# Roy-Kid/ADMP

Hardware: AMD Instinct MI355X
Metric: ns/day (electrostatics get_forces per 1 fs step, polarizable PME incl. SCF, moving atoms) (higher is better)
Workload: dtype f64; 1 GPU; water_pol_1024 (BASELINE configs[1]): 1024 polarizable MPID waters = 3072 atoms, seeded liquid box L=31.289 A, rc 4 A, f64; n_atoms=3072, n_pairs=42510, pair_list=fixed during the timed steps, parallelism=single GPU

## Files before the change

admp_amd/_lib.py:

```python
import ctypes

import numpy as np
import os

_HERE = os.path.dirname(os.path.abspath(__file__))
LIB_PATH = os.environ.get('ADMP_HIP_LIB') or os.path.join(_HERE, 'lib', 'libadmp_hip.so')

_c = ctypes
_vp, _i32, _i64, _dbl = _c.c_void_p, _c.c_int, _c.c_int64, _c.c_double
_dp = _c.POINTER(_c.c_double)
_ip = _c.POINTER(_c.c_int)

PROTOTYPES = {
    'admp_version': (_c.c_char_p, []),
    'admp_create': (_i32, [_c.POINTER(_vp), _i32, _i32]),
    'admp_destroy': (_i32, [_vp]),
    'admp_last_error': (_c.c_char_p, [_vp]),
    'admp_set_stream': (_i32, [_vp, _vp]),
    'admp_use_default_stream': (_i32, [_vp]),
    'admp_synchronize': (_i32, [_vp]),
    'admp_set_topology': (_i32, [_vp, _i32, _vp, _vp, _vp, _vp, _vp]),
    'admp_set_ewald': (_i32, [_vp, _dbl, _i32, _i32, _i32, _i32, _i32]),
    'admp_set_pairs': (_i32, [_vp, _i64, _vp, _i32]),
    'admp_share_neighbors': (_i32, [_vp, _vp]),
# ... 15 lines not shown
    'admp_pair_program_build': (_i32, [_vp, _c.c_char_p, _i32, _ip]),
    'admp_pair_program_energy_grad': (_i32, [_vp, _i32, _vp, _dp, _vp, _i32, _dp, _dp, _vp, _i32]),
    'admp_disp_param_grad': (_i32, [_vp, _vp, _dp, _vp, _i32, _i32, _dp, _vp]),
    'admp_tt_param_grad': (_i32, [_vp, _vp, _dp, _vp, _i32, _dp, _vp]),
    'admp_thole_sums': (_i32, [_vp, _vp, _dp, _vp, _vp, _vp, _i32, _dp, _dp, _vp, _vp, _vp]),
    'admp_pscale_grad': (_i32, [_vp, _vp, _dp, _vp, _vp, _vp, _i32, _dp, _dp, _vp, _dp]),
    'admp_mscale_grad': (_i32, [_vp, _i32, _vp, _dp, _vp, _i32, _i32, _dp, _i32]),
    'admp_md_bonded': (_i32, [_vp, _vp, _dp, _i32, _vp, _vp, _i32, _vp, _vp, _vp, _vp]),
    'admp_md_kick_drift': (_i32, [_vp, _i32, _vp, _vp, _vp, _vp, _dbl, _dbl, _vp]),
    'admp_neighbor_count': (_i32, [_vp, _i32, _vp, _dp, _dbl, _c.POINTER(_i64)]),
    'admp_neighbor_fill': (_i32, [_vp, _vp]),
    'admp_set_pairs_from_positions': (_i32, [_vp, _vp, _dp, _dbl]),
    'admp_slab_configure': (_i32, [_vp, _i32, _i32]),
    'admp_slab_info': (_i32, [_vp, _c.POINTER(_i64)]),
    'admp_scf_stats': (_i32, [_vp, _c.POINTER(_i64), _i32]),
    'admp_set_comm': (_i32, [_vp, _vp]),
    'admp_slab_home': (_i32, [_vp, _vp, _ip, _ip]),
    'admp_rccl_unique_id': (_i32, [_vp]),
    'admp_rccl_create': (_i32, [_c.POINTER(_vp), _i32, _vp, _i32, _i32]),
    'admp_rccl_destroy': (_i32, [_vp]),
    'admp_rccl_abort': (_i32, [_vp]),
    'admp_rccl_stats': (_i32, [_vp, _c.POINTER(_i64), _c.POINTER(_i64), _i32]),
    'admp_rccl_all_reduce': (_i32, [_vp, _vp, _i64, _i32, _i32, _vp]),
    'admp_rccl_all_to_all_v': (_i32, [_vp, _vp, _c.POINTER(_i64), _vp, _c.POINTER(_i64), _i32, _vp]),
    'admp_rccl_shift': (_i32, [_vp, _vp, _vp, _i64, _i32, _i32, _vp]),
    'admp_rccl_version': (_i32, [_ip]),
    'admp_rccl_last_error': (_c.c_char_p, []),
    'admp_set_comm_rccl': (_i32, [_vp, _vp]),
    'admp_profile_enable': (_i32, [_vp, _i32]),
    'admp_profile_filter': (_i32, [_vp, _c.c_char_p]),
# ... 58 lines not shown
```

admp_amd/csrc/dft_kernels.hip:

```cpp
#include "dft_lines.h"
#include "env.h"

namespace admp {

int dft_tile_cols(int N) { return dft_cols(N, dft_kq(), 0, 0); }
template <class T, int KQ, int JS>
__global__ __launch_bounds__(kDftBlock) void k_dft_z_r2c(int N, int nlines, int NL, int TK, const T* __restrict__ mesh,
                                                        Cx<T>* __restrict__ spec, const Cx<T>* __restrict__ twg,
                                                        long mesh_stride, long spec_stride) {
  mesh += blockIdx.y * mesh_stride;
  spec += blockIdx.y * spec_stride;
  const int H = (N - 1) / 2, Kh = N / 2 + 1;
  Cx<T>* tw = reinterpret_cast<Cx<T>*>(dft_smem);
  Cx<T>* p = tw + N;
  T* x0 = reinterpret_cast<T*>(p + H * NL);
  T* xn = x0 + NL;
  const int line0 = blockIdx.x * NL;
  const int nl = min(NL, nlines - line0);
  for (int t = threadIdx.x; t < N; t += kDftBlock) tw[t] = twg[t];
  for (int t = threadIdx.x; t < H * nl; t += kDftBlock) {
    const int l = t / H, jj = t - l * H;
    const T* x = mesh + (long)(line0 + l) * N;
    const T a = x[1 + jj], b = x[N - 1 - jj];
    p[jj * NL + l] = Cx<T>{a + b, a - b};
// ... 108 lines not shown
    dft_pair_outputs_js<T, SIGN, KQ, JS>(N, k, NC, ab + c, x0[c], xn[c], tw, half, Xk, Xnk);
#pragma unroll
    for (int q = 0; q < KQ; ++q) {
      const int kq = g + q * TK;
      if (kq < Kh) {
        if (JS == 1 || half == 0) spec[base + (long)kq * jstride + c] = Xk[q];
        if ((JS == 1 || half == 1) && kq != 0 && 2 * kq != N) spec[base + (long)(N - kq) * jstride + c] = Xnk[q];
      }
    }
  }
}

template <class T, int KQ, int JS>
__global__ __launch_bounds__(kDftBlock) void k_dft_x_conv(XConvArgs<T> xa) {
  dft_x_conv_body<T, KQ, JS>(xa, blockIdx.x, blockIdx.y, blockIdx.z);
}

template <class T, int KQ, int JS, int NTP>
__global__ __launch_bounds__(kDftBlock) void k_dft_x_mix(int N, int ncols, int NC, int TK, long jstride, long fixstride,
                                                        int K3, Cx<T>* __restrict__ spec, DftTabs<T> tabs, MixTab mix,
                                                        const Cx<T>* __restrict__ twg, double* energies, int slot,
                                                        long spec_tstride) {
  const int H = (N - 1) / 2, Kh = N / 2 + 1, NCt = NC / NTP;
  PairCx<T>* ab = reinterpret_cast<PairCx<T>*>(dft_smem);
  Cx<T>* tw = reinterpret_cast<Cx<T>*>(ab + H * NC);
  Cx<T>* x0 = tw + N;
  Cx<T>* xn = x0 + NC;
  Cx<T>* S = xn + NC;
  const int col0 = blockIdx.x * NCt;
  const int ncp = min(NCt, ncols - col0);
// ... 463 lines not shown
    KQ_SWITCH((k_dft_strided<T, -1, KQ, JS><<<grid, kDftBlock, sh, st>>>(N, Kh, NC, TK, (long)Kh, (long)K[1] * Kh, sp, t1, ss)))
  }
}
template <class T>
void launch_dft_x_conv(hipStream_t st, const int K[3], const T* tw, T* spec, const DftTabs<T>& tabs, double* energies,
                       int slot, int nb, long spec_stride) {
  const int N = K[0], Kh = K[2] / 2 + 1, H = (N - 1) / 2, TK = dft_tasks(N, dft_kq());
  const int NC = dft_cols(N, dft_kq(), sizeof(PairCx<T>) * (size_t)H + sizeof(Cx<T>) * (size_t)(2 + N), sizeof(Cx<T>) * (size_t)N);
  const size_t sh = sizeof(PairCx<T>) * (size_t)(H * NC) + sizeof(Cx<T>) * (size_t)(N + 2 * NC + N * NC);
  const dim3 grid((Kh + NC - 1) / NC, K[1], nb);
  const XConvArgs<T> xa{N, Kh, NC, TK, (long)K[1] * Kh, (long)Kh, K[2], reinterpret_cast<Cx<T>*>(spec), tabs,
                        reinterpret_cast<const Cx<T>*>(tw), energies, slot, spec_stride / 2};
  KQ_SWITCH((k_dft_x_conv<T, KQ, JS><<<grid, kDftBlock, sh, st>>>(xa)))
}
template <class T>
void launch_dft_x_mix(hipStream_t st, const int K[3], const T* tw, T* spec, const DftTabs<T>& tabs, const MixTab& mix,
                      long spec_stride, double* energies, int slot) {
  const int N = K[0], Kh = K[2] / 2 + 1, H = (N - 1) / 2, TK = dft_tasks(N, dft_kq());
  const int ntp = mix.nt <= 1 ? 1 : (mix.nt == 2 ? 2 : 4);
  int NC = dft_cols(N, dft_kq(), sizeof(PairCx<T>) * (size_t)H + sizeof(Cx<T>) * (size_t)(2 + N), sizeof(Cx<T>) * (size_t)N);
  NC -= NC % ntp;
  if (NC < ntp) NC = ntp;
  const int NCt = NC / ntp;
  const size_t sh = sizeof(PairCx<T>) * (size_t)(H * NC) + sizeof(Cx<T>) * (size_t)(N + 2 * NC + N * NC);
  const dim3 grid((Kh + NCt - 1) / NCt, K[1], 1);
#define XMIX(NTP)                                                                                                          \
  k_dft_x_mix<T, 2, 1, NTP><<<grid, kDftBlock, sh, st>>>(N, Kh, NC, TK, (long)K[1] * Kh, (long)Kh, K[2],                    \
                                                         reinterpret_cast<Cx<T>*>(spec), tabs, mix,                        \
                                                         reinterpret_cast<const Cx<T>*>(tw), energies, slot, spec_stride / 2)
  if (ntp == 1) XMIX(1); else if (ntp == 2) XMIX(2); else XMIX(4);
// ... 33 lines not shown
  }
  auto kern = k_dft_zy_fwd<T, 2, false>;
  if (attr_set[0] < sh) { (void)hipFuncSetAttribute((const void*)kern, hipFuncAttributeMaxDynamicSharedMemorySize, (int)sh); attr_set[0] = sh; }
  kern<<<grid, kZyBlock, sh, st>>>(K[1], K[2], mesh, reinterpret_cast<Cx<T>*>(spec), t1, t2, mesh_stride, spec_stride / 2,
                                   PlaneSpread<T>());
  return false;
}
#undef KQ_SWITCH
#define INST(T)                                                                                   \
  template bool dft_zy_fits<T>(const int*);                                                       \
  template bool dft_zy_spread_fits<T>(const int*, int);                                           \
  template bool launch_dft_zy<T>(hipStream_t, const int*, const T*, T*, T*, int, int, long, long, T*, const PlaneSpread<T>*); \
  template bool launch_dft_z<T>(hipStream_t, const int*, const T*, T*, T*, int, int, long, long, T*); \
  template void launch_dft_y<T>(hipStream_t, const int*, const T*, T*, int, int, long);           \
  template void launch_dft_x_conv<T>(hipStream_t, const int*, const T*, T*, const DftTabs<T>&, double*, int, int, long); \
  template void launch_dft_x_mix<T>(hipStream_t, const int*, const T*, T*, const DftTabs<T>&, const MixTab&, long, double*, int);
INST(float)
INST(double)
#undef INST

}
```

admp_amd/csrc/dft_lines.h:

```cpp
#pragma once
#include "dft_math.h"
#include "launch.h"
#include "reduce.h"

namespace admp {

#ifndef ADMP_DFT_BLOCK
#define ADMP_DFT_BLOCK 256
#endif
constexpr int kDftBlock = ADMP_DFT_BLOCK;
constexpr size_t kDftLdsBudget = 60 * 1024;

static inline int dft_kq() { return 2; }
static inline int dft_js() { return 1; }
static inline int dft_tasks(int N, int KQ) { return (N / 2 + 1 + KQ - 1) / KQ; }
static inline int dft_cols(int N, int KQ, size_t bytes_per_col, size_t fixed_bytes) {
  int nc = (kDftBlock / dft_js()) / dft_tasks(N, KQ);
  if (nc < 1) nc = 1;
  while (nc > 1 && fixed_bytes + bytes_per_col * nc > kDftLdsBudget) --nc;
  return nc;
}

extern __shared__ __align__(32) unsigned char dft_smem[];

// ... 59 lines not shown
    xn[c] = b;
  }
}

template <class T>
struct XConvArgs {
  int N, ncols, NC, TK;
  long jstride, fixstride;
  int K3;
  Cx<T>* spec;
  DftTabs<T> tabs;
  const Cx<T>* twg;
  double* energies;
  int slot;
  long spec_stride;
};
template <class T, int KQ, int JS>
__device__ __forceinline__ void dft_x_conv_body(const XConvArgs<T>& xa, int bx, int by, int bz) {
  const int N = xa.N, ncols = xa.ncols, NC = xa.NC, TK = xa.TK, K3 = xa.K3, slot = xa.slot;
  const long jstride = xa.jstride, fixstride = xa.fixstride;
  const Cx<T>* __restrict__ twg = xa.twg;
  double* energies = xa.energies;
  Cx<T>* __restrict__ spec = xa.spec + bz * xa.spec_stride;
  const T* __restrict__ gtab = xa.tabs.p[bz];
  const int H = (N - 1) / 2, Kh = N / 2 + 1;
  PairCx<T>* ab = reinterpret_cast<PairCx<T>*>(dft_smem);
  Cx<T>* tw = reinterpret_cast<Cx<T>*>(ab + H * NC);
  Cx<T>* x0 = tw + N;
  Cx<T>* xn = x0 + NC;
  Cx<T>* S = xn + NC;
// ... 82 lines not shown
    Cx<T> Xk[KQ], Xnk[KQ];
    dft_pair_outputs_js<T, +1, KQ, JS>(N, k, NC, ab + c, x0[c], xn[c], tw, half, Xk, Xnk);
#pragma unroll
    for (int q = 0; q < KQ; ++q) {
      const int kq = g + q * TK;
      if (kq < Kh) {
        if (JS == 1 || half == 0) spec[base + (long)kq * jstride + c] = Xk[q];
        if ((JS == 1 || half == 1) && kq != 0 && 2 * kq != N) spec[base + (long)(N - kq) * jstride + c] = Xnk[q];
      }
    }
  }
  e = block_reduce_sum<kDftBlock>(e);
  if (threadIdx.x == 0) atomicAdd(&energies[slot], e);
}

}
```

admp_amd/csrc/dft_math.h:

```cpp
#pragma once
#include "pme_math.h"

namespace admp {

template <class T>
struct alignas(2 * sizeof(T)) Cx {
  T re, im;
};
template <class T>
struct alignas(4 * sizeof(T)) PairCx {
  T are, aim, bre, bim;
};

constexpr int kDftReseed = 8;

template <class T>
ADMP_HD Cx<T> cx_mul(Cx<T> a, Cx<T> b) {
  return Cx<T>{a.re * b.re - a.im * b.im, a.re * b.im + a.im * b.re};
}

template <class T>
struct TwStep {
  Cx<T> w, aux;
  T t;
// ... 175 lines not shown

template <class T, int KQ>
ADMP_HD void irdft_pair_outputs(int N, const int* j, int stride, const Cx<T>* p, T X0re, T Xnre, const Cx<T>* tw, T* xj,
                                T* xnj) {
  T P[KQ], R[KQ];
  real_pair_sums<T, KQ>(N, j, stride, p, tw, P, R);
#pragma unroll
  for (int q = 0; q < KQ; ++q) {
    T base = X0re + T(2) * P[q];
    if ((N & 1) == 0) base += (j[q] & 1) ? -Xnre : Xnre;
    xj[q] = base - T(2) * R[q];
    xnj[q] = base + T(2) * R[q];
  }
}

inline int largest_prime_factor(int n) {
  int best = 1;
  for (int p = 2; (long)p * p <= n; ++p)
    while (n % p == 0) {
      best = p;
      n /= p;
    }
  return n > 1 ? (n > best ? n : best) : best;
}

}
```

admp_amd/csrc/engine.hip:

```cpp
#include <hip/hip_runtime.h>
#include <hip/hiprtc.h>
#include <rocfft/rocfft.h>

#include <algorithm>
#include <cmath>
#include <cstdio>
#include <cstring>
#include <map>
#include <memory>
#include <mutex>
#include <set>
#include <string>
#include <functional>
#include <vector>

#include "../../include/admp_hip.h"
#include "dft_math.h"
#include "launch.h"
#include "rccl_comm.h"
#include "scf_policy.h"

using namespace admp;

namespace {
// ... 132 lines not shown
  void c_all_reduce(void* buf, int64_t n, int dtype, int op, int tag) {
    const int rc = rccl ? rccl_all_reduce(rccl, stream, buf, n, dtype, op, tag) : comm.all_reduce(comm.ctx, buf, n, dtype, op, tag);
    if (rc != 0) comm_fail("all_reduce", rc);
  }
  void c_all_to_all_v(const void* send, const int64_t* sc, void* recv, const int64_t* rc_, int dtype, int tag) {
    const int rc = rccl ? rccl_all_to_all_v(rccl, stream, send, sc, recv, rc_, dtype, tag)
                        : comm.all_to_all_v(comm.ctx, send, sc, recv, rc_, dtype, tag);
    if (rc != 0) comm_fail("all_to_all_v", rc);
  }
  void c_shift(const void* send, void* recv, int64_t n, int dtype, int to_next, int tag) {
    const int rc = rccl ? rccl_shift(rccl, stream, send, recv, n, dtype, to_next, tag)
                        : comm.shift(comm.ctx, send, recv, n, dtype, to_next, tag);
    if (rc != 0) comm_fail("shift", rc);
  }
  int64_t scf_stats[8] = {0, 0, 0, 0, 0, 0, 0, 0};
  const void* U_src = nullptr;
  const void* U_src_now = nullptr;
  double cutoff = 0.0;
  int ref_korder = 0;
  int keep_pol_sites = 0;
  int side_stream_on = 1;
  virtual void after_error() {}
  long nbr_gen = 0;
  NbrTable nbr_full;
  bool pruned = false;
  void unprune() {
    if (!pruned) return;
    nbr = nbr_full;
    nbr_full = NbrTable();
    pruned = false;
// ... 347 lines not shown
  const IndTable& wind() const { return cut_on ? cut_ind : ind; }
  long act_gen = 0, act_top_na = -1;
  int act_n = -1;
  bool act_fresh = false;
  long ind_nbr_gen = -1, ind_act_gen = -1;
  long eval_seq = 0, ind_bins_eval = -1, ind_bins_gen = -1;
  int ind_bins_n = -1;
  const int* ind_bins_at = nullptr;
  DevBuf dft_tw;
  DevBuf bases_d;
  bool use_dft = false;
  bool use_pfa = false;
  PfaPlan pfa;
  DevBuf pfa_tw, pfa_fmap, pfa_ptab, gtab_nat;
  struct TabKey { double box[9] = {0}, kappa = -1; int K[3] = {0, 0, 0}, Y0 = 0, ref = 0; bool pfa = false; } tabkey[4];
  static int tab_slot(int which) { return which == 1 ? 0 : (which == 6 ? 1 : (which == 8 ? 2 : 3)); }
  static_assert(kScfChainSteps == E_CHAIN, "one residual word per chained Jacobi step");
  ScfHistory scf;
  bool mono_ok = false;

  ~Engine() override {
    destroy_plans();
    for (DevBuf* b : {&sites, &grad, &pot, &fld_pair, &fld_recip, &field, &energies_d, &s_pos, &s_Q, &s_pol,
                      &s_thole, &s_U, &s_out, &s_dQ, &s_par, &mesh, &spec, &gtabs[0], &gtabs[1], &gtabs[2], &gtabs[3], &fft_work, &binv_d, &scan_scratch, &bin_cells,
                      &bin_sorted, &bin_scan, &home_list, &dft_tw, &bases_d, &vir_d, &act_d, &isites, &mesh2, &act_tmp,
                      &rq_d, &pfa_tw, &pfa_fmap, &pfa_ptab, &gtab_nat, &fx_tw, &bin_cells_ind, &bin_sorted_ind, &srow_d, &onehot_d, &tcount_d, &prune_rowptr, &prune_cnt, &prune_col,
                      &cut_end, &cut_col, &cut_iend, &cut_icol})
      b->release();
    free_topology();
    if (ind.end) (void)hipFree(ind.end);
    if (ind.col) (void)hipFree(ind.col);
    cells.release();
    sl.release();
    free_programs();
    if (Eh) (void)hipHostFree(Eh);
    prof.destroy();
    if (side) { (void)hipStreamSynchronize(side); (void)hipStreamDestroy(side); }
    if (ev_fork) (void)hipEventDestroy(ev_fork);
    if (ev_join) (void)hipEventDestroy(ev_join);
    if (own_stream && stream) (void)hipStreamDestroy(stream);
  }

// ... 404 lines not shown
      { TIMED("dft_z_c2r"); launch_pfa_z<T>(stream, pfa, tw, mesh_p, spec_p, 1); }
      return false;
    }
    if (use_dft) {
      const T* tw = dft_tw.as<T>();
      const bool planes = dft_zy_fits<T>(K);
      ARG_CHECK(!sp || planes, "internal: plane spread without the plane kernels");
      if (planes && sp) { TIMED("dft_spread_zy_fwd"); launch_dft_zy<T>(stream, K, tw, mesh_p, spec_p, 0, 1, 0, 0, nullptr, sp); }
      else if (planes) { TIMED("dft_zy_fwd"); launch_dft_zy<T>(stream, K, tw, mesh_p, spec_p, 0); }
      else {
        { TIMED("dft_z_r2c"); launch_dft_z<T>(stream, K, tw, mesh_p, spec_p, 0); }
        { TIMED("dft_y_fwd"); launch_dft_y<T>(stream, K, tw, spec_p, 0); }
      }
      DftTabs<T> tabs;
      tabs.p[0] = gtab;
      if (rider && rider->kind) { TIMED("dft_x_kspace"); launch_dft_x_conv_rider<T>(stream, K, tw, spec_p, tabs, Ed, slot, *rider); }
      else { TIMED("dft_x_kspace"); launch_dft_x_conv<T>(stream, K, tw, spec_p, tabs, Ed, slot); }
      bool added;
      if (planes) { TIMED("dft_yz_inv"); added = launch_dft_zy<T>(stream, K, tw, mesh_p, spec_p, 1, 1, 0, 0, accum); }
      else {
        { TIMED("dft_y_inv"); launch_dft_y<T>(stream, K, tw, spec_p, 1); }
        { TIMED("dft_z_c2r"); added = launch_dft_z<T>(stream, K, tw, mesh_p, spec_p, 1, 1, 0, 0, accum); }
      }
      return added;
    }
    if (use_fx) {
      run_plan("rocfft_r2c_yz", plan2_f, mesh_p, spec_p);
      { TIMED("fftx_kspace"); launch_fftx_conv<T>(stream, K, fx_tw.as<T>(), spec_p, gtab, Ed, slot, fx_khp); }
      run_plan("rocfft_c2r_yz", plan2_b, spec_p, mesh_o);
      return false;
    }
// ... 84 lines not shown
    gtab_cur = buf.template as<T>();
    bool same = key.kappa == kappa && key.K[0] == K[0] && key.K[1] == K[1] && key.K[2] == K[2] &&
                key.Y0 == (snranks > 1 ? Y0 : 0) && key.ref == ref_korder && key.pfa == use_pfa;
    for (int k = 0; k < 9 && same; ++k) same = key.box[k] == box[k];
    if (same) return;
    HIP_TRY(hipMemcpyAsync(binv_d.p, inv, 9 * sizeof(double), hipMemcpyHostToDevice, stream));
    HIP_TRY(hipStreamSynchronize(stream));
    {
      TIMED("gtab");
      launch_gtab<T>(stream, K, snranks > 1 ? Y0 : 0, nyown(), binv_d.as<double>(), std::fabs(vol), kappa, which, gtab_cur, ref_korder,
                     use_pfa ? pfa_fmap.as<int>() : nullptr, use_pfa ? pfa.Khp : 0);
    }
    std::memcpy(key.box, box, sizeof(key.box));
    key.kappa = kappa; key.K[0] = K[0]; key.K[1] = K[1]; key.K[2] = K[2]; key.Y0 = snranks > 1 ? Y0 : 0; key.ref = ref_korder;
    key.pfa = use_pfa;
  }

  ScaleTab<T> make_tab(int ns, const double* mS, const double* pS) {
    ARG_CHECK(ns >= 1 && mS, "mScales missing");
    ScaleTab<T> t;
    for (int nb = 0; nb < 16; ++nb) {
      int idx = ((nb - 1) % ns + ns) % ns;
      t.mm[nb] = (T)(mS[idx] - 1.0);
      double p = pS ? pS[idx] : 0.0;
      t.p[nb] = (T)p;
      t.w0[nb] = (T)(1.0 / (std::exp((p - 1e-3) / 1e-5) + 1.0));
    }
    return t;
  }

// ... 1862 lines not shown
int admp_set_dipole_source(admp_handle* h, const void* U_init) {
  return guarded(h, [&](EngineBase& e) { e.U_src = U_init; });
}
int admp_set_cutoff(admp_handle* h, double rc) {
  return guarded(h, [&](EngineBase& e) {
    ARG_CHECK(rc >= 0.0, "negative cutoff");
    e.cutoff = rc;
  });
}
int admp_scf_stats(admp_handle* h, int64_t* out8, int reset) {
  return guarded(h, [&](EngineBase& e) {
    ARG_CHECK(out8, "null");
    for (int k = 0; k < 8; ++k) { out8[k] = e.scf_stats[k]; if (reset) e.scf_stats[k] = 0; }
  });
}
int admp_slab_home(admp_handle* h, int32_t* home_out, int* n_home, int* n_import) {
  return guarded(h, [&](EngineBase& e) { e.slab_home(home_out, n_home, n_import); });
}

int admp_profile_enable(admp_handle* h, int on) {
  return guarded(h, [&](EngineBase& e) { e.prof.collect(e.stream); e.prof.on = on != 0; });
}
int admp_profile_filter(admp_handle* h, const char* label) {
  return guarded(h, [&](EngineBase& e) { e.prof.only = label ? label : ""; });
}
int admp_profile_reset(admp_handle* h) {
  return guarded(h, [&](EngineBase& e) { e.prof.reset(e.stream); });
}
int admp_profile_count(admp_handle* h) {
  if (!h || !h->eng) return ADMP_E_ARG;
// ... 15 lines not shown
```

admp_amd/csrc/launch.h:

```cpp
#pragma once
#include <hip/hip_runtime.h>
#include <stdint.h>

#include <initializer_list>

#include "env.h"
#include "frame_math.h"
#include "pme_math.h"
#include "spline_math.h"

namespace admp {

template <class T>
struct ScaleTab {
  T mm[16];
  T p[16];
  T w0[16];
};

struct NbrTable {
  int* rowptr = nullptr;
  int* col = nullptr;
  int* rowend = nullptr;
  int64_t n_half = 0;
// ... 129 lines not shown
template <class T>
bool dft_zy_spread_fits(const int K[3], int na);
template <class T>
bool launch_dft_zy(hipStream_t st, const int K[3], const T* tw, T* mesh, T* spec, int inverse, int nb = 1, long mesh_stride = 0,
                   long spec_stride = 0, T* accum = nullptr, const PlaneSpread<T>* sp = nullptr );
template <class T>
bool launch_dft_z(hipStream_t st, const int K[3], const T* tw, T* mesh, T* spec, int inverse, int nb = 1,
                  long mesh_stride = 0, long spec_stride = 0,
                  T* accum = nullptr );
template <class T>
void launch_dft_y(hipStream_t st, const int K[3], const T* tw, T* spec, int inverse, int nb = 1,
                  long spec_stride = 0);
template <class T>
void launch_dft_x_conv(hipStream_t st, const int K[3], const T* tw, T* spec, const DftTabs<T>& tabs, double* energies,
                       int slot, int nb = 1, long spec_stride = 0);

struct PfaAxis { int N, N1, N2; };
struct PfaPlan {
  PfaAxis ax[3];
  int Khp;
  int tw_off[3];
  const int* ptab[3];
};
bool pfa_split(int N, PfaAxis* out);
void pfa_index_table(const PfaAxis& a, int* t);
void pfa_freq_of_slot(const PfaAxis& a, int* f);
void pfa_freq_of_zcolumn(const PfaAxis& a, int* f);
template <class T>
void launch_pfa_z(hipStream_t st, const PfaPlan& p, const T* tw, T* mesh, T* spec, int inverse, int nb = 1, long mesh_stride = 0,
                  long spec_stride = 0);
// ... 51 lines not shown
  unsigned nblocks = 0, grid = 0;
  const int* n_dev = nullptr;
  const int* cls_flags = nullptr;
  const RQ4<T>* rq = nullptr;
  const T* tholes = nullptr;
};
template <class T>
bool field_rider_full(FieldRider<T>& r, int na, const NbrTable& nb, const Site<T>* sites, const Box<T>& box,
                      const ScaleTab<T>& tab, T kappa, T* fld, const int* rows, const int* n_dev, const int* cls_flags,
                      const RQ4<T>* rq, const T* tholes);
template <class T>
bool field_rider_ind(FieldRider<T>& r, int n_rows, const IndTable& it, const Site<T>* sites, const Box<T>& box,
                     const ScaleTab<T>& tab, T kappa, T* fld, const int* rows);
template <class T>
void launch_dft_x_conv_rider(hipStream_t st, const int K[3], const T* tw, T* spec, const DftTabs<T>& tabs, double* energies,
                             int slot, const FieldRider<T>& fr);
template <class T>
int prune_table(hipStream_t st, int na, const NbrTable& full, const T* pos, const Box<T>& box, double rc, int* rowptr_out,
                int* cnt, int* col_out, void** scratch, size_t* scratch_bytes, int64_t* total);
template <class T>
int build_cut_table(hipStream_t st, int n, const int* rows, const NbrTable& nb, const Site<T>* sites, const Box<T>& box,
                    double rc, int* end_out, int* col_out, int* iend, int* icol);
int sort_ints(hipStream_t st, int* keys, int* keys_tmp, int n, void** scratch, size_t* scratch_bytes);
template <class T>
int build_ind_table(hipStream_t st, int na, const NbrTable& nb, const Site<T>* sites, IndTable& it);
int pair_lanes_per_row(int n_rows);
template <class T>
void launch_thole_sums(hipStream_t st, int na, const NbrTable& nb, const Site<T>* sites, const Box<T>& box,
                       const ScaleTab<T>& tab, T* sumX, T* sumXw, const int* rows = nullptr, int n_rows = 0);
template <class T>
void launch_mscale_sums(hipStream_t st, int kind, int na, const NbrTable& nb, const Site<T>* sites, const T* pos,
// ... 223 lines not shown
```

admp_amd/csrc/pair_kernels.hip:

```cpp
#include <cstdlib>

#include "disp_math.h"
#include "dft_lines.h"
#include "launch.h"
#include "reduce.h"

namespace admp {

constexpr int kPairBlock = 256;
#ifndef ADMP_FULL_BLOCK
#define ADMP_FULL_BLOCK 256
#endif
constexpr int kFullBlock = ADMP_FULL_BLOCK;

template <class T, int LPR>
__device__ __forceinline__ T row_reduce(T v) {
#pragma unroll
  for (int off = LPR / 2; off > 0; off >>= 1) v += __shfl_xor(v, off, 64);
  return v;
}

template <class T>
__device__ __forceinline__ void stage_tab(const ScaleTab<T>& tab, T* s) {
  if (threadIdx.x < 16) {
// ... 203 lines not shown
  }
#pragma unroll
  for (int q = 0; q < 3; ++q) F[q] = row_reduce<T, LPR>(F[q]);
  if (row >= 0 && sub == 0) { fld[3 * row] += F[0]; fld[3 * row + 1] += F[1]; fld[3 * row + 2] += F[2]; }
}
template <class T, int LPR>
__global__ __launch_bounds__(kPairBlock) void k_pair_field_ind(int na, const int* __restrict__ irow,
                                                               const int* __restrict__ iend,
                                                               const int* __restrict__ icol,
                                                               const Site<T>* __restrict__ sites, Box<T> box,
                                                               ScaleTab<T> tab, T kappa, T* __restrict__ fld,
                                                               const int* __restrict__ rows) {
  pair_field_ind_block<T, LPR>(blockIdx.x, na, irow, iend, icol, sites, box, tab, kappa, fld, rows);
}

template <class T, int LPR, bool CUT>
__global__ __launch_bounds__(kPairBlock) void k_xconv_pair(XConvArgs<T> xa, FieldRider<T> fr, int nbx) {
  static_assert(kPairBlock == kDftBlock, "the two kinds of workgroups share one launch");
  if ((int)blockIdx.x < nbx) {
    dft_x_conv_body<T, 2, 1>(xa, blockIdx.x, blockIdx.y, 0);
    return;
  }
  const unsigned bid = (blockIdx.x - (unsigned)nbx) * gridDim.y + blockIdx.y;
  if (bid >= fr.grid) return;
  if (fr.kind == 1)
    pair_field_block<T, LPR, CUT>(bid, fr.na, fr.rowptr, fr.rowend, fr.col, fr.sites, fr.box, fr.tab, fr.kappa, fr.fld, fr.rows, fr.nblocks,
                             fr.n_dev, fr.cls_flags, fr.rq, fr.tholes);
  else
    pair_field_ind_block<T, LPR>(bid, fr.na, fr.rowptr, fr.rowend, fr.col, fr.sites, fr.box, fr.tab, fr.kappa, fr.fld, fr.rows);
}

template <class T>
__global__ __launch_bounds__(256) void k_pack_scalar_rows(int na, int np, const T* __restrict__ pos, const T* __restrict__ par,
                                                          SRow<T>* __restrict__ rows) {
  const int i = blockIdx.x * 256 + threadIdx.x;
// ... 463 lines not shown
  r.kappa = kappa; r.fld = fld; r.rows = rows; r.nblocks = grid_for(na, kRiderLpr); r.grid = xcd_grid(r.nblocks);
  r.n_dev = n_dev; r.cls_flags = cls_flags; r.rq = rq; r.tholes = tholes;
  return true;
}
template <class T>
bool field_rider_ind(FieldRider<T>& r, int n_rows, const IndTable& it, const Site<T>* sites, const Box<T>& box,
                     const ScaleTab<T>& tab, T kappa, T* fld, const int* rows) {
  if (n_rows <= 0 || field_lanes_per_row(n_rows, true) != kRiderLpr) return false;
  r.kind = 2; r.na = n_rows; r.rowptr = it.beg; r.rowend = it.end; r.col = it.col; r.sites = sites; r.box = box; r.tab = tab;
  r.kappa = kappa; r.fld = fld; r.rows = rows; r.nblocks = grid_for(n_rows, kRiderLpr); r.grid = xcd_grid(r.nblocks);
  r.n_dev = nullptr; r.cls_flags = nullptr; r.rq = nullptr; r.tholes = nullptr;
  return true;
}
template <class T>
void launch_dft_x_conv_rider(hipStream_t st, const int K[3], const T* tw, T* spec, const DftTabs<T>& tabs, double* energies,
                             int slot, const FieldRider<T>& fr) {
  const int N = K[0], Kh = K[2] / 2 + 1, H = (N - 1) / 2, TK = dft_tasks(N, dft_kq());
  const int NC = dft_cols(N, dft_kq(), sizeof(PairCx<T>) * (size_t)H + sizeof(Cx<T>) * (size_t)(2 + N), sizeof(Cx<T>) * (size_t)N);
  const size_t sh = sizeof(PairCx<T>) * (size_t)(H * NC) + sizeof(Cx<T>) * (size_t)(N + 2 * NC + N * NC);
  const int nbx = (Kh + NC - 1) / NC;
  const unsigned extra = (fr.grid + (unsigned)K[1] - 1) / (unsigned)K[1];
  const XConvArgs<T> xa{N, Kh, NC, TK, (long)K[1] * Kh, (long)Kh, K[2], reinterpret_cast<Cx<T>*>(spec), tabs,
                        reinterpret_cast<const Cx<T>*>(tw), energies, slot, 0};
  const dim3 grid((unsigned)nbx + extra, (unsigned)K[1], 1);
  if (fr.kind == 1 && fr.rowend) k_xconv_pair<T, kRiderLpr, true><<<grid, kPairBlock, sh, st>>>(xa, fr, nbx);
  else k_xconv_pair<T, kRiderLpr, false><<<grid, kPairBlock, sh, st>>>(xa, fr, nbx);
}

template <class T>
void launch_pair_field_ind(hipStream_t st, int n_rows, const IndTable& it, const Site<T>* sites, const Box<T>& box,
                           const ScaleTab<T>& tab, T kappa, T* fld, const int* rows) {
  if (n_rows <= 0) return;
  const int lpr = field_lanes_per_row(n_rows, true);
#define CALL(L)                                                                                                          \
  k_pair_field_ind<T, L><<<xcd_grid(grid_for(n_rows, L)), kPairBlock, 0, st>>>(n_rows, it.beg, it.end, it.col, sites, box, tab, \
                                                                               kappa, fld, rows)
  ADMP_LPR_SWITCH(lpr, CALL)
#undef CALL
}
template <class T>
void launch_disp_pair(hipStream_t st, int na, const NbrTable& nb, const SRow<T>* srows, const Box<T>& box,
// ... 33 lines not shown

#define INST(T)                                                                                                     \
  template void launch_pair_full<T>(hipStream_t, int, const NbrTable&, const Site<T>*, const Box<T>&,               \
                                    const ScaleTab<T>&, T, int, T*, T*, double*, const int*, T*, int, const int*,   \
                                    const RQ4<T>*, const T*);                                                       \
  template void launch_pair_field<T>(hipStream_t, int, const NbrTable&, const Site<T>*, const Box<T>&,              \
                                     const ScaleTab<T>&, T, T*, const int*, const int*, const int*,                 \
                                     const RQ4<T>*, const T*);                                                      \
  template void launch_pair_field_ind<T>(hipStream_t, int, const IndTable&, const Site<T>*, const Box<T>&,          \
                                         const ScaleTab<T>&, T, T*, const int*);                                    \
  template bool field_rider_full<T>(FieldRider<T>&, int, const NbrTable&, const Site<T>*, const Box<T>&, const ScaleTab<T>&, \
                                    T, T*, const int*, const int*, const int*, const RQ4<T>*, const T*);            \
  template bool field_rider_ind<T>(FieldRider<T>&, int, const IndTable&, const Site<T>*, const Box<T>&,             \
                                   const ScaleTab<T>&, T, T*, const int*);                                          \
  template void launch_dft_x_conv_rider<T>(hipStream_t, const int*, const T*, T*, const DftTabs<T>&, double*, int,  \
                                           const FieldRider<T>&);                                                   \
  template void launch_pack_scalar_rows<T>(hipStream_t, int, int, const T*, const T*, SRow<T>*);                    \
  template void launch_disp_pair<T>(hipStream_t, int, const NbrTable&, const SRow<T>*, const Box<T>&,               \
                                    const ScaleTab<T>&, T, int, T*, double*, const int*, int, double);              \
  template void launch_tt_pair<T>(hipStream_t, int, const NbrTable&, const SRow<T>*, const Box<T>&,                 \
                                  const ScaleTab<T>&, T*, double*, const int*, int, double);                        \
  template void launch_mscale_sums<T>(hipStream_t, int, int, const NbrTable&, const Site<T>*, const T*, const T*,   \
                                      const Box<T>&, int, double*, double, const int*, int);                        \
  template void launch_thole_sums<T>(hipStream_t, int, const NbrTable&, const Site<T>*, const Box<T>&,              \
                                     const ScaleTab<T>&, T*, T*, const int*, int);                                  \
  template void launch_pair_virial<T>(hipStream_t, int, const NbrTable&, const Site<T>*, const Box<T>&,             \
                                      const ScaleTab<T>&, T, int, double*, const int*, int);                        \
  template void launch_scalar_pair_virial<T>(hipStream_t, int, int, const NbrTable&, const T*, const T*,            \
                                             const Box<T>&, const ScaleTab<T>&, T, int, double*, double,            \
                                             const int*, int);                                                      \
  template void launch_scalar_pair_pgrad<T>(hipStream_t, int, int, const NbrTable&, const T*, const T*,             \
// ... 7 lines not shown
```

admp_amd/pme.py:

```python
import ctypes
import math
import warnings

import numpy as np
import torch

from . import _lib, settings
from ._device import HipForceBase

DIELECTRIC = 1389.35455846
DEFAULT_THOLE_WIDTH = 0.3


def setup_ewald_parameters(rc, ethresh, box):
    box = np.asarray(box.detach().cpu() if isinstance(box, torch.Tensor) else box, dtype=np.float64)
    kappa = math.sqrt(-math.log(2 * ethresh)) / rc
    K1 = math.ceil(2 * kappa * box[0, 0] / 3 / ethresh ** 0.2)
    K2 = math.ceil(2 * kappa * box[1, 1] / 3 / ethresh ** 0.2)
    K3 = math.ceil(2 * kappa * box[2, 2] / 3 / ethresh ** 0.2)
    if settings.FFT_FRIENDLY_MESH:
        K1, K2, K3 = (next_smooth(int(k)) for k in (K1, K2, K3))
    return kappa, int(K1), int(K2), int(K3)


# ... 334 lines not shown
                                      self._ptr(pol_t), self._ptr(th_t), len(mS), _lib.darr(mS), _lib.darr(pS), self._ptr(U),
                                      out)
        _lib.check(self._h, rc, 'admp_pscale_grad')
        return np.array(out[:], dtype=np.float64)

    def get_mscale_gradient(self, positions, box, pairs, Q_local, mScales):
        return self._mscale_gradient(0, positions, box, pairs, self._pad_Q(Q_local), 9, len(self._host64(mScales)))

    def scf_stats(self, reset=False):
        out = (ctypes.c_int64 * 8)()
        _lib.check(self._h, self._L.admp_scf_stats(self._h, out, 1 if reset else 0), 'admp_scf_stats')
        keys = ('plain', 'speculative', 'speculative_failed', 'chained', 'chained_too_short', 'chained_too_long',
                'wasted_increments', 'jacobi_steps')
        return dict(zip(keys, (int(v) for v in out)))

    def optimize_Uind(self, positions, box, pairs, Q_local, pol, tholes, mScales, pScales, dScales, U_init=None,
                      maxiter=None, thresh=None):
        if not self.lpol:
            raise RuntimeError('optimize_Uind needs lpol=True')
        r = self._evaluate(positions, box, pairs, Q_local, mScales, pol, tholes, pScales, dScales, U_init,
                           want_grad=False, maxiter=maxiter, thresh=thresh)
        self._warn_unconverged(r)
        return self._like(r['U'], positions), r['flag'], r['i']
```

include/admp_hip.h:

```cpp
#ifndef ADMP_HIP_H
#define ADMP_HIP_H

#include <stdint.h>

#ifdef __cplusplus
extern "C" {
#endif

typedef struct admp_handle admp_handle;

enum {
  ADMP_OK = 0,
  ADMP_E_ARG = -1,
  ADMP_E_HIP = -2,
  ADMP_E_FFT = -3,
  ADMP_E_NOGPU = -4,
  ADMP_E_STATE = -5,
  ADMP_E_COMM = -6
};

const char* admp_version(void);

int admp_create(admp_handle** out, int device, int precision );
int admp_destroy(admp_handle* h);
// ... 101 lines not shown
int admp_rccl_unique_id(void* out128);
int admp_rccl_create(admp_rccl** out, int device, const void* id128, int rank, int nranks);
int admp_rccl_destroy(admp_rccl* c);
int admp_rccl_abort(admp_rccl* c);
int admp_rccl_stats(admp_rccl* c, int64_t* bytes_out, int64_t* calls_out, int reset);
int admp_rccl_all_reduce(admp_rccl* c, void* buf, int64_t count, int dtype , int op , void* hip_stream);
int admp_rccl_all_to_all_v(admp_rccl* c, const void* send, const int64_t* send_counts, void* recv, const int64_t* recv_counts,
                           int dtype, void* hip_stream);
int admp_rccl_shift(admp_rccl* c, const void* send, void* recv, int64_t count, int dtype, int to_next, void* hip_stream);
int admp_rccl_version(int* version);
const char* admp_rccl_last_error(void);
int admp_set_comm_rccl(admp_handle* h, admp_rccl* c);
int admp_slab_home(admp_handle* h, int32_t* home_out, int* n_home, int* n_import);

int admp_scf_stats(admp_handle* h, int64_t* out8, int reset);

int admp_profile_enable(admp_handle* h, int on);
int admp_profile_filter(admp_handle* h, const char* label);
int admp_profile_reset(admp_handle* h);
int admp_profile_count(admp_handle* h);
int admp_profile_entry(admp_handle* h, int idx, const char** label, double* total_ms, int64_t* launches);

#ifdef __cplusplus
}
#endif
#endif
```

Before: 469.1 ns/day.

## Replace x-axis DFT convolution with precomputed circulant table when Green's function is even

```diff
diff --git a/admp_amd/_lib.py b/admp_amd/_lib.py
--- a/admp_amd/_lib.py
+++ b/admp_amd/_lib.py
@@ -53,6 +53,7 @@
     'admp_slab_configure': (_i32, [_vp, _i32, _i32]),
     'admp_slab_info': (_i32, [_vp, _c.POINTER(_i64)]),
     'admp_scf_stats': (_i32, [_vp, _c.POINTER(_i64), _i32]),
+    'admp_xpass_stats': (_i32, [_vp, _c.POINTER(_i64), _i32]),
     'admp_set_comm': (_i32, [_vp, _vp]),
     'admp_slab_home': (_i32, [_vp, _vp, _ip, _ip]),
     'admp_rccl_unique_id': (_i32, [_vp]),
diff --git a/admp_amd/csrc/dft_kernels.hip b/admp_amd/csrc/dft_kernels.hip
--- a/admp_amd/csrc/dft_kernels.hip
+++ b/admp_amd/csrc/dft_kernels.hip
@@ -146,6 +146,26 @@
 template <class T, int KQ, int JS>
 __global__ __launch_bounds__(kDftBlock) void k_dft_x_conv(XConvArgs<T> xa) {
   dft_x_conv_body<T, KQ, JS>(xa, blockIdx.x, blockIdx.y, blockIdx.z);
+}
+
+template <class T, int KQ>
+__global__ __launch_bounds__(kDftBlock) void k_dft_x_circ(XConvArgs<T> xa) {
+  dft_x_circ_body<T, KQ>(xa, blockIdx.x, blockIdx.y);
+}
+template <class T>
+__global__ __launch_bounds__(256) void k_ctab(int N, long ncol, const T* __restrict__ gtab, T* __restrict__ ctab, int* uneven) {
+  double* cw = reinterpret_cast<double*>(dft_smem);
+  for (int m = threadIdx.x; m < N; m += 256) cw[m] = circ_cos(m, N);
+  __syncthreads();
+  const long t = (long)blockIdx.x * 256 + threadIdx.x;
+  if (t >= ncol * (N / 2 + 1)) return;
+  const int d = (int)(t / ncol);
+  const T* __restrict__ G = gtab + (t - (long)d * ncol);
+  const double c = circ_table_entry(N, d, (double)G[0], [=](int k) { return (double)G[k * ncol] + (double)G[(N - k) * ncol]; },
+                                    (N & 1) ? 0.0 : (double)G[(N / 2) * ncol], [=](int m) { return cw[m]; });
+  ctab[t] = (T)c;
+  if (d == 0 && !circ_column_even(N, [=](int k) { return (double)G[k * ncol]; }, sizeof(T) == 4 ? 0x1p-24 : 0x1p-53))
+    atomicOr(uneven, 1);
 }
 
 template <class T, int KQ, int JS, int NTP>
@@ -639,6 +659,22 @@
   KQ_SWITCH((k_dft_x_conv<T, KQ, JS><<<grid, kDftBlock, sh, st>>>(xa)))
 }
 template <class T>
+void launch_dft_x_circ(hipStream_t st, const int K[3], T* spec, const T* ctab, double* energies, int slot) {
+  const int N = K[0], Kh = K[2] / 2 + 1, TK = dft_tasks(N, dft_kq());
+  const int NC = dft_cols(N, dft_kq(), dft_x_circ_col_bytes<T>(N), 0);
+  const size_t sh = dft_x_circ_col_bytes<T>(N) * (size_t)NC;
+  const dim3 grid((Kh + NC - 1) / NC, K[1], 1);
+  XConvArgs<T> xa{N, Kh, NC, TK, (long)K[1] * Kh, (long)Kh, K[2], reinterpret_cast<Cx<T>*>(spec), DftTabs<T>(), nullptr,
+                  energies, slot, 0};
+  xa.ctab = ctab;
+  k_dft_x_circ<T, 2><<<grid, kDftBlock, sh, st>>>(xa);
+}
+template <class T>
+void launch_ctab(hipStream_t st, const int K[3], const T* gtab, T* ctab, int* uneven) {
+  const long ncol = (long)K[1] * (K[2] / 2 + 1), n = ncol * (K[0] / 2 + 1);
+  k_ctab<T><<<(unsigned)((n + 255) / 256), 256, sizeof(double) * (size_t)K[0], st>>>(K[0], ncol, gtab, ctab, uneven);
+}
+template <class T>
 void launch_dft_x_mix(hipStream_t st, const int K[3], const T* tw, T* spec, const DftTabs<T>& tabs, const MixTab& mix,
                       long spec_stride, double* energies, int slot) {
   const int N = K[0], Kh = K[2] / 2 + 1, H = (N - 1) / 2, TK = dft_tasks(N, dft_kq());
@@ -702,6 +738,8 @@
   template bool launch_dft_z<T>(hipStream_t, const int*, const T*, T*, T*, int, int, long, long, T*); \
   template void launch_dft_y<T>(hipStream_t, const int*, const T*, T*, int, int, long);           \
   template void launch_dft_x_conv<T>(hipStream_t, const int*, const T*, T*, const DftTabs<T>&, double*, int, int, long); \
+  template void launch_dft_x_circ<T>(hipStream_t, const int*, T*, const T*, double*, int);       \
+  template void launch_ctab<T>(hipStream_t, const int*, const T*, T*, int*);                      \
   template void launch_dft_x_mix<T>(hipStream_t, const int*, const T*, T*, const DftTabs<T>&, const MixTab&, long, double*, int);
 INST(float)
 INST(double)
diff --git a/admp_amd/csrc/dft_lines.h b/admp_amd/csrc/dft_lines.h
--- a/admp_amd/csrc/dft_lines.h
+++ b/admp_amd/csrc/dft_lines.h
@@ -97,6 +97,7 @@
   double* energies;
   int slot;
   long spec_stride;
+  const T* ctab = nullptr;
 };
 template <class T, int KQ, int JS>
 __device__ __forceinline__ void dft_x_conv_body(const XConvArgs<T>& xa, int bx, int by, int bz) {
@@ -209,4 +210,59 @@
   if (threadIdx.x == 0) atomicAdd(&energies[slot], e);
 }
 
-}
+template <class T>
+inline size_t dft_x_circ_col_bytes(int N) {
+  return sizeof(PairCx<T>) * (size_t)((N - 1) / 2) + 2 * sizeof(Cx<T>) + sizeof(T) * (size_t)circ_ext_len(N);
+}
+template <class T, int KQ>
+__device__ __forceinline__ void dft_x_circ_body(const XConvArgs<T>& xa, int bx, int by) {
+  const bool ENERGY = xa.slot != E_SCRATCH;
+  const int N = xa.N, ncols = xa.ncols, NC = xa.NC, TK = xa.TK, K3 = xa.K3;
+  const long jstride = xa.jstride;
+  Cx<T>* __restrict__ spec = xa.spec;
+  const T* __restrict__ ctab = xa.ctab;
+  const int H = (N - 1) / 2, Kh = N / 2 + 1;
+  PairCx<T>* ab = reinterpret_cast<PairCx<T>*>(dft_smem);
+  Cx<T>* x0 = reinterpret_cast<Cx<T>*>(ab + H * NC);
+  Cx<T>* xn = x0 + NC;
+  T* cext = reinterpret_cast<T*>(xn + NC);
+  const int col0 = bx * NC;
+  const int nca = min(NC, ncols - col0);
+  const long base = (long)by * xa.fixstride + col0;
+  for (int t = threadIdx.x; t < Kh * NC; t += kDftBlock) {
+    const int d = t / NC, cc = t - d * NC;
+    const T v = cc < nca ? ctab[base + (long)d * jstride + cc] : T(0);
+    cext[(N / 2 + d) * NC + cc] = v;
+    cext[(N / 2 - d) * NC + cc] = v;
+    if (N - d <= N / 2 + H) cext[(N / 2 + N - d) * NC + cc] = v;
+  }
+  load_pairs<T>(N, NC, nca, spec, base, jstride, ab, x0, xn);
+  __syncthreads();
+  const int g = (int)threadIdx.x / NC, c = (int)threadIdx.x - g * NC;
+  double e = 0.0;
+  if (g < TK && c < nca) {
+    int i[KQ];
+#pragma unroll
+    for (int q = 0; q < KQ; ++q) i[q] = (g + q * TK < Kh) ? g + q * TK : 0;
+    Cx<T> P[KQ], M[KQ];
+    circ_pair_outputs<T, KQ>(N, i, NC, cext + (N / 2) * NC + c, NC, ab + c, x0[c], xn[c], P, M);
+#pragma unroll
+    for (int q = 0; q < KQ; ++q) {
+      const int iq = g + q * TK;
+      if (iq < Kh) {
+        const bool single = iq == 0 || 2 * iq == N;
+        if (ENERGY) e += circ_pair_energy<T>(N, iq, P[q], M[q], ab[(single ? 0 : iq - 1) * NC + c], x0[c], xn[c]);
+        spec[base + (long)iq * jstride + c] = Cx<T>{T(0.5) * (P[q].re + M[q].re), T(0.5) * (P[q].im + M[q].im)};
+        if (!single) spec[base + (long)(N - iq) * jstride + c] = Cx<T>{T(0.5) * (P[q].re - M[q].re), T(0.5) * (P[q].im - M[q].im)};
+      }
+    }
+    const int kz = col0 + c;
+    if (ENERGY && (kz == 0 || ((K3 & 1) == 0 && kz == K3 / 2))) e *= 0.5;
+  }
+  if (ENERGY) {
+    e = block_reduce_sum<kDftBlock>(e);
+    if (threadIdx.x == 0) atomicAdd(&xa.energies[xa.slot], e);
+  }
+}
+
+}
diff --git a/admp_amd/csrc/dft_math.h b/admp_amd/csrc/dft_math.h
--- a/admp_amd/csrc/dft_math.h
+++ b/admp_amd/csrc/dft_math.h
@@ -213,6 +213,91 @@
   }
 }
 
+
+ADMP_HD double circ_cos(int m, int N) {
+  if (2 * m > N) m = N - m;
+  const double pi = 3.141592653589793;
+  return 4 * m > N ? -cos(pi * (double)(N - 2 * m) / (double)N) : cos(pi * (double)(2 * m) / (double)N);
+}
+template <class LoadGs, class CosM>
+ADMP_HD double circ_table_entry(int N, int d, double G0, LoadGs gs, double Gn, CosM cosm) {
+  const int H = (N - 1) / 2;
+  double c = G0;
+  int m = 0;
+  for (int k = 1; k <= H; ++k) {
+    m += d;
+    if (m >= N) m -= N;
+    c += gs(k) * cosm(m);
+  }
+  if ((N & 1) == 0) c += (d & 1) ? -Gn : Gn;
+  return c;
+}
+constexpr double kCircEvenUlps = 8.0;
+template <class LoadG>
+ADMP_HD bool circ_column_even(int N, LoadG G, double ulp) {
+  const int H = (N - 1) / 2;
+  double gmax = fabs(G(0));
+  for (int k = 1; k < N; ++k) { const double g = fabs(G(k)); gmax = g > gmax ? g : gmax; }
+  bool ok = true;
+  for (int k = 1; k <= H; ++k) ok = ok && fabs(G(k) - G(N - k)) <= kCircEvenUlps * ulp * gmax;
+  return ok;
+}
+ADMP_HD int circ_ext_len(int N) { return N / 2 + N / 2 + (N - 1) / 2 + 1; }
+ADMP_HD int circ_fold(int e, int N) {
+  if (e < 0) e = -e;
+  return 2 * e > N ? N - e : e;
+}
+
+template <class T>
+ADMP_HD void circ_step(const PairCx<T>& p, T c1, T c2, Cx<T>& P, Cx<T>& M) {
+  const T s = c1 + c2, d = c1 - c2;
+  P.re += s * p.are;
+  P.im += s * p.aim;
+  M.re += d * p.bre;
+  M.im += d * p.bim;
+}
+constexpr int kCircUnroll = 4;
+template <class T, int KQ>
+ADMP_HD void circ_pair_outputs(int N, const int* i, int cstride, const T* ce, int stride, const PairCx<T>* ab, Cx<T> x0,
+                               Cx<T> xn, Cx<T>* P, Cx<T>* M) {
+  const int H = (N - 1) / 2;
+  const T* cm[KQ];
+  const T* cp[KQ];
+#pragma unroll
+  for (int q = 0; q < KQ; ++q) {
+    const T c0 = T(2) * ce[i[q] * cstride];
+    P[q] = Cx<T>{c0 * x0.re, c0 * x0.im};
+    M[q] = Cx<T>{T(0), T(0)};
+    if ((N & 1) == 0) {
+      const T cn = T(2) * ce[(i[q] - N / 2) * cstride];
+      P[q].re += cn * xn.re;
+      P[q].im += cn * xn.im;
+    }
+    cm[q] = ce + (i[q] - 1) * cstride;
+    cp[q] = ce + (i[q] + 1) * cstride;
+  }
+  int j = 0;
+  for (; j + kCircUnroll <= H; j += kCircUnroll) {
+#pragma unroll
+    for (int jj = 0; jj < kCircUnroll; ++jj) {
+      const PairCx<T> p = ab[(j + jj) * stride];
+#pragma unroll
+      for (int q = 0; q < KQ; ++q) circ_step(p, cm[q][-(j + jj) * cstride], cp[q][(j + jj) * cstride], P[q], M[q]);
+    }
+  }
+  for (; j < H; ++j) {
+    const PairCx<T> p = ab[j * stride];
+#pragma unroll
+    for (int q = 0; q < KQ; ++q) circ_step(p, cm[q][-j * cstride], cp[q][j * cstride], P[q], M[q]);
+  }
+}
+template <class T>
+ADMP_HD double circ_pair_energy(int N, int i, Cx<T> P, Cx<T> M, const PairCx<T>& ai, Cx<T> x0, Cx<T> xn) {
+  if (i == 0) return 0.5 * ((double)x0.re * P.re + (double)x0.im * P.im);
+  if (2 * i == N) return 0.5 * ((double)xn.re * P.re + (double)xn.im * P.im);
+  return 0.5 * ((double)ai.are * P.re + (double)ai.aim * P.im + (double)ai.bre * M.re + (double)ai.bim * M.im);
+}
+
 inline int largest_prime_factor(int n) {
   int best = 1;
   for (int p = 2; (long)p * p <= n; ++p)
diff --git a/admp_amd/csrc/engine.hip b/admp_amd/csrc/engine.hip
--- a/admp_amd/csrc/engine.hip
+++ b/admp_amd/csrc/engine.hip
@@ -170,6 +170,7 @@
     if (rc != 0) comm_fail("shift", rc);
   }
   int64_t scf_stats[8] = {0, 0, 0, 0, 0, 0, 0, 0};
+  int64_t xpass_stats[2] = {0, 0};
   const void* U_src = nullptr;
   const void* U_src_now = nullptr;
   double cutoff = 0.0;
@@ -547,6 +548,9 @@
   PfaPlan pfa;
   DevBuf pfa_tw, pfa_fmap, pfa_ptab, gtab_nat;
   struct TabKey { double box[9] = {0}, kappa = -1; int K[3] = {0, 0, 0}, Y0 = 0, ref = 0; bool pfa = false; } tabkey[4];
+  DevBuf xctab, xctab_flag;
+  bool xctab_ok = false;
+  static bool xcirc_on() { static const bool on = env_flag("ADMP_DFT_XCIRC", true); return on; }
   static int tab_slot(int which) { return which == 1 ? 0 : (which == 6 ? 1 : (which == 8 ? 2 : 3)); }
   static_assert(kScfChainSteps == E_CHAIN, "one residual word per chained Jacobi step");
   ScfHistory scf;
@@ -558,7 +562,7 @@
                       &s_thole, &s_U, &s_out, &s_dQ, &s_par, &mesh, &spec, &gtabs[0], &gtabs[1], &gtabs[2], &gtabs[3], &fft_work, &binv_d, &scan_scratch, &bin_cells,
                       &bin_sorted, &bin_scan, &home_list, &dft_tw, &bases_d, &vir_d, &act_d, &isites, &mesh2, &act_tmp,
                       &rq_d, &pfa_tw, &pfa_fmap, &pfa_ptab, &gtab_nat, &fx_tw, &bin_cells_ind, &bin_sorted_ind, &srow_d, &onehot_d, &tcount_d, &prune_rowptr, &prune_cnt, &prune_col,
-                      &cut_end, &cut_col, &cut_iend, &cut_icol})
+                      &cut_end, &cut_col, &cut_iend, &cut_icol, &xctab, &xctab_flag})
       b->release();
     free_topology();
     if (ind.end) (void)hipFree(ind.end);
@@ -993,7 +997,10 @@
       }
       DftTabs<T> tabs;
       tabs.p[0] = gtab;
-      if (rider && rider->kind) { TIMED("dft_x_kspace"); launch_dft_x_conv_rider<T>(stream, K, tw, spec_p, tabs, Ed, slot, *rider); }
+      const T* ct = xctab_ok && gtab == gtabs[0].template as<T>() ? xctab.template as<T>() : nullptr;
+      ++xpass_stats[ct ? 0 : 1];
+      if (rider && rider->kind) { TIMED("dft_x_kspace"); launch_dft_x_conv_rider<T>(stream, K, tw, spec_p, tabs, Ed, slot, *rider, ct); }
+      else if (ct) { TIMED("dft_x_kspace"); launch_dft_x_circ<T>(stream, K, spec_p, ct, Ed, slot); }
       else { TIMED("dft_x_kspace"); launch_dft_x_conv<T>(stream, K, tw, spec_p, tabs, Ed, slot); }
       bool added;
       if (planes) { TIMED("dft_yz_inv"); added = launch_dft_zy<T>(stream, K, tw, mesh_p, spec_p, 1, 1, 0, 0, accum); }
@@ -1108,6 +1115,19 @@
     std::memcpy(key.box, box, sizeof(key.box));
     key.kappa = kappa; key.K[0] = K[0]; key.K[1] = K[1]; key.K[2] = K[2]; key.Y0 = snranks > 1 ? Y0 : 0; key.ref = ref_korder;
     key.pfa = use_pfa;
+    if (slot == 0) {
+      xctab_ok = false;
+      if (use_dft && !use_pfa && snranks == 1 && xcirc_on()) {
+        xctab.need((size_t)(K[0] / 2 + 1) * K[1] * (K[2] / 2 + 1) * sizeof(T));
+        xctab_flag.need(sizeof(int));
+        HIP_TRY(hipMemsetAsync(xctab_flag.p, 0, sizeof(int), stream));
+        { TIMED("xcirc_table"); launch_ctab<T>(stream, K, gtab_cur, xctab.as<T>(), xctab_flag.as<int>()); }
+        int uneven = 1;
+        HIP_TRY(hipMemcpyAsync(&uneven, xctab_flag.p, sizeof(int), hipMemcpyDeviceToHost, stream));
+        HIP_TRY(hipStreamSynchronize(stream));
+        xctab_ok = uneven == 0;
+      }
+    }
   }
 
   ScaleTab<T> make_tab(int ns, const double* mS, const double* pS) {
@@ -3000,6 +3020,12 @@
     for (int k = 0; k < 8; ++k) { out8[k] = e.scf_stats[k]; if (reset) e.scf_stats[k] = 0; }
   });
 }
+int admp_xpass_stats(admp_handle* h, int64_t* out2, int reset) {
+  return guarded(h, [&](EngineBase& e) {
+    ARG_CHECK(out2, "null");
+    for (int k = 0; k < 2; ++k) { out2[k] = e.xpass_stats[k]; if (reset) e.xpass_stats[k] = 0; }
+  });
+}
 int admp_slab_home(admp_handle* h, int32_t* home_out, int* n_home, int* n_import) {
   return guarded(h, [&](EngineBase& e) { e.slab_home(home_out, n_home, n_import); });
 }
diff --git a/admp_amd/csrc/launch.h b/admp_amd/csrc/launch.h
--- a/admp_amd/csrc/launch.h
+++ b/admp_amd/csrc/launch.h
@@ -167,6 +167,10 @@
 template <class T>
 void launch_dft_x_conv(hipStream_t st, const int K[3], const T* tw, T* spec, const DftTabs<T>& tabs, double* energies,
                        int slot, int nb = 1, long spec_stride = 0);
+template <class T>
+void launch_dft_x_circ(hipStream_t st, const int K[3], T* spec, const T* ctab, double* energies, int slot);
+template <class T>
+void launch_ctab(hipStream_t st, const int K[3], const T* gtab, T* ctab, int* uneven);
 
 struct PfaAxis { int N, N1, N2; };
 struct PfaPlan {
@@ -248,7 +252,7 @@
                      const ScaleTab<T>& tab, T kappa, T* fld, const int* rows);
 template <class T>
 void launch_dft_x_conv_rider(hipStream_t st, const int K[3], const T* tw, T* spec, const DftTabs<T>& tabs, double* energies,
-                             int slot, const FieldRider<T>& fr);
+                             int slot, const FieldRider<T>& fr, const T* ctab = nullptr );
 template <class T>
 int prune_table(hipStream_t st, int na, const NbrTable& full, const T* pos, const Box<T>& box, double rc, int* rowptr_out,
                 int* cnt, int* col_out, void** scratch, size_t* scratch_bytes, int64_t* total);
diff --git a/admp_amd/csrc/pair_kernels.hip b/admp_amd/csrc/pair_kernels.hip
--- a/admp_amd/csrc/pair_kernels.hip
+++ b/admp_amd/csrc/pair_kernels.hip
@@ -241,11 +241,12 @@
   pair_field_ind_block<T, LPR>(blockIdx.x, na, irow, iend, icol, sites, box, tab, kappa, fld, rows);
 }
 
-template <class T, int LPR, bool CUT>
+template <class T, int LPR, bool CUT, bool CIRC>
 __global__ __launch_bounds__(kPairBlock) void k_xconv_pair(XConvArgs<T> xa, FieldRider<T> fr, int nbx) {
   static_assert(kPairBlock == kDftBlock, "the two kinds of workgroups share one launch");
   if ((int)blockIdx.x < nbx) {
-    dft_x_conv_body<T, 2, 1>(xa, blockIdx.x, blockIdx.y, 0);
+    if (CIRC) dft_x_circ_body<T, 2>(xa, blockIdx.x, blockIdx.y);
+    else dft_x_conv_body<T, 2, 1>(xa, blockIdx.x, blockIdx.y, 0);
     return;
   }
   const unsigned bid = (blockIdx.x - (unsigned)nbx) * gridDim.y + blockIdx.y;
@@ -739,17 +740,26 @@
 }
 template <class T>
 void launch_dft_x_conv_rider(hipStream_t st, const int K[3], const T* tw, T* spec, const DftTabs<T>& tabs, double* energies,
-                             int slot, const FieldRider<T>& fr) {
+                             int slot, const FieldRider<T>& fr, const T* ctab) {
   const int N = K[0], Kh = K[2] / 2 + 1, H = (N - 1) / 2, TK = dft_tasks(N, dft_kq());
-  const int NC = dft_cols(N, dft_kq(), sizeof(PairCx<T>) * (size_t)H + sizeof(Cx<T>) * (size_t)(2 + N), sizeof(Cx<T>) * (size_t)N);
-  const size_t sh = sizeof(PairCx<T>) * (size_t)(H * NC) + sizeof(Cx<T>) * (size_t)(N + 2 * NC + N * NC);
+  const int NC = ctab ? dft_cols(N, dft_kq(), dft_x_circ_col_bytes<T>(N), 0)
+                      : dft_cols(N, dft_kq(), sizeof(PairCx<T>) * (size_t)H + sizeof(Cx<T>) * (size_t)(2 + N), sizeof(Cx<T>) * (size_t)N);
+  const size_t sh = ctab ? dft_x_circ_col_bytes<T>(N) * (size_t)NC
+                         : sizeof(PairCx<T>) * (size_t)(H * NC) + sizeof(Cx<T>) * (size_t)(N + 2 * NC + N * NC);
   const int nbx = (Kh + NC - 1) / NC;
   const unsigned extra = (fr.grid + (unsigned)K[1] - 1) / (unsigned)K[1];
-  const XConvArgs<T> xa{N, Kh, NC, TK, (long)K[1] * Kh, (long)Kh, K[2], reinterpret_cast<Cx<T>*>(spec), tabs,
-                        reinterpret_cast<const Cx<T>*>(tw), energies, slot, 0};
+  XConvArgs<T> xa{N, Kh, NC, TK, (long)K[1] * Kh, (long)Kh, K[2], reinterpret_cast<Cx<T>*>(spec), tabs,
+                  reinterpret_cast<const Cx<T>*>(tw), energies, slot, 0};
+  xa.ctab = ctab;
   const dim3 grid((unsigned)nbx + extra, (unsigned)K[1], 1);
-  if (fr.kind == 1 && fr.rowend) k_xconv_pair<T, kRiderLpr, true><<<grid, kPairBlock, sh, st>>>(xa, fr, nbx);
-  else k_xconv_pair<T, kRiderLpr, false><<<grid, kPairBlock, sh, st>>>(xa, fr, nbx);
+  const bool cut = fr.kind == 1 && fr.rowend;
+  if (ctab) {
+    if (cut) k_xconv_pair<T, kRiderLpr, true, true><<<grid, kPairBlock, sh, st>>>(xa, fr, nbx);
+    else k_xconv_pair<T, kRiderLpr, false, true><<<grid, kPairBlock, sh, st>>>(xa, fr, nbx);
+  } else {
+    if (cut) k_xconv_pair<T, kRiderLpr, true, false><<<grid, kPairBlock, sh, st>>>(xa, fr, nbx);
+    else k_xconv_pair<T, kRiderLpr, false, false><<<grid, kPairBlock, sh, st>>>(xa, fr, nbx);
+  }
 }
 
 template <class T>
@@ -813,7 +823,7 @@
   template bool field_rider_ind<T>(FieldRider<T>&, int, const IndTable&, const Site<T>*, const Box<T>&,             \
                                    const ScaleTab<T>&, T, T*, const int*);                                          \
   template void launch_dft_x_conv_rider<T>(hipStream_t, const int*, const T*, T*, const DftTabs<T>&, double*, int,  \
-                                           const FieldRider<T>&);                                                   \
+                                           const FieldRider<T>&, const T*);                                         \
   template void launch_pack_scalar_rows<T>(hipStream_t, int, int, const T*, const T*, SRow<T>*);                    \
   template void launch_disp_pair<T>(hipStream_t, int, const NbrTable&, const SRow<T>*, const Box<T>&,               \
                                     const ScaleTab<T>&, T, int, T*, double*, const int*, int, double);              \
diff --git a/admp_amd/pme.py b/admp_amd/pme.py
--- a/admp_amd/pme.py
+++ b/admp_amd/pme.py
@@ -372,6 +372,11 @@
                 'wasted_increments', 'jacobi_steps')
         return dict(zip(keys, (int(v) for v in out)))
 
+    def xpass_stats(self, reset=False):
+        out = (ctypes.c_int64 * 2)()
+        _lib.check(self._h, self._L.admp_xpass_stats(self._h, out, 1 if reset else 0), 'admp_xpass_stats')
+        return {'circulant': int(out[0]), 'transforms': int(out[1])}
+
     def optimize_Uind(self, positions, box, pairs, Q_local, pol, tholes, mScales, pScales, dScales, U_init=None,
                       maxiter=None, thresh=None):
         if not self.lpol:
diff --git a/include/admp_hip.h b/include/admp_hip.h
--- a/include/admp_hip.h
+++ b/include/admp_hip.h
@@ -139,6 +139,7 @@
 int admp_slab_home(admp_handle* h, int32_t* home_out, int* n_home, int* n_import);
 
 int admp_scf_stats(admp_handle* h, int64_t* out8, int reset);
+int admp_xpass_stats(admp_handle* h, int64_t* out2, int reset);
 
 int admp_profile_enable(admp_handle* h, int on);
 int admp_profile_filter(admp_handle* h, const char* label);
```

Measured after the change: 489.5 ns/day, median of 6. +4.4%, better.
